# XuyangBai/PointDSC

Hardware: NVIDIA B200
Metric: correspondence-sets/sec (PointDSC.forward, N=1000, B=256) (higher is better)
Workload: dtype fp16 hi/lo split (3 products) with f32 accumulate

## Files before the change

pointdsc_b200/csrc/encoder_tc.cu:

```cuda
#include <cuda_bf16.h>
#include <cuda_fp16.h>
#include <cuda_runtime.h>

#include <cmath>
#include <cstdlib>
#include <cstring>
#include <vector>

#include "common.cuh"
#include "encoder_tc.h"
#include "kernels.h"
#include "tc_attention.cuh"
#include "tc_attention_p.cuh"
#include "tc_chain.cuh"
#include "tc_common.cuh"
#include "tc_ptx.cuh"

namespace pdsc {

template <int FMT>
static void build_image(const float* W, int rows, int K, double scale, uint8_t* dst) {
  const int panels = K / 64;
  const size_t panel_bytes = (size_t)rows * 128;
  uint8_t* hi = dst;
  uint8_t* lo = dst + panels * panel_bytes;
  for (int r = 0; r < rows; ++r)
    for (int k = 0; k < K; ++k) {
      const float x = (float)((double)W[(size_t)r * K + k] * scale);
      const uint16_t h = to_16<FMT>(x);
      const uint16_t l = to_16<FMT>(x - from_16<FMT>(h));
      const size_t off = (size_t)(k / 64) * panel_bytes + sw128_offset((uint32_t)r, (uint32_t)(k % 64));
      std::memcpy(hi + off, &h, 2);
      std::memcpy(lo + off, &l, 2);
    }
}

template <int FMT>
static void build_layer(const TcLayerHost& L, uint8_t* base) {
  build_image<FMT>(L.w1, 128, 128, 1.0, base + kW1);
  build_image<FMT>(L.wq, 128, 128, (double)kQScale, base + kWq);
  build_image<FMT>(L.wk, 128, 128, 1.0, base + kWk);
  build_image<FMT>(L.wv, 128, 128, 1.0, base + kWv);
  build_image<FMT>(L.wm0, 64, 128, 1.0, base + kWm0);
  build_image<FMT>(L.wm1, 64, 64, 1.0, base + kWm1);
  build_image<FMT>(L.wm2, 128, 64, 1.0, base + kWm2);
}

int tc_build_weights(const TcLayerHost* layers, int num_layers, TcWeights* out) {
  tc_free_weights(out);
  const size_t per_fmt = (size_t)num_layers * kLayerBytes;
  std::vector<uint8_t> host(2 * per_fmt, 0);
  for (int fmt = 0; fmt < 2; ++fmt)
    for (int l = 0; l < num_layers; ++l) {
      uint8_t* base = host.data() + fmt * per_fmt + (size_t)l * kLayerBytes;
      const TcLayerHost& L = layers[l];
      if (fmt == kFmtF16) build_layer<kFmtF16>(L, base); else build_layer<kFmtBF16>(L, base);
      float* b = reinterpret_cast<float*>(base + kBias);
      for (int i = 0; i < 128; ++i) {
        b[kB1 + i] = L.b1[i];
        b[kBq + i] = (float)((double)L.bq[i] * (double)kQScale);
        b[kBk + i] = L.bk[i];
        b[kBv + i] = L.bv[i];
        b[kBm2 + i] = L.bm2[i];
      }
      for (int i = 0; i < 64; ++i) {
        b[kBm0 + i] = L.bm0[i];
        b[kBm1 + i] = L.bm1[i];
      }
    }
  cudaError_t err = cudaMalloc(&out->arena, host.size());
  if (err != cudaSuccess) return (int)err;
  err = cudaMemcpy(out->arena, host.data(), host.size(), cudaMemcpyHostToDevice);
  if (err != cudaSuccess) return (int)err;
  out->arena_bytes = host.size();
  out->num_layers = num_layers;
  return 0;
}

void tc_free_weights(TcWeights* w) {
  if (w->arena) cudaFree(w->arena);
  w->arena = nullptr;
  w->arena_bytes = 0;
}

static inline int q_tiles(int N) { return (N + 127) / 128; }
static inline int k_tiles(int N) { return (N + 63) / 64; }

constexpr int kAttnSplitMaxItems = 320;
constexpr size_t kAttnSplitBytes = (size_t)kAttnSplitMaxItems * (65536 + 1024);

size_t tc_scratch_bytes(int B, int N) {
  return ((size_t)B * q_tiles(N) + (size_t)B * k_tiles(N)) * 65536 + 1024 + kAttnSplitBytes;
}

static void attn_split_policy(int B, int N, int num_sms, int* splits, int* TS) {
  const int QT = q_tiles(N), KT = k_tiles(N);
  *splits = 1;
  *TS = KT;
  if (2 * B * QT > num_sms || KT < 4) return;
  const int want = (num_sms + QT - 1) / QT;
  int ts = (KT + want - 1) / want;
  if (ts < 2) ts = 2;
  const int sp = (KT + ts - 1) / ts;
  if (sp < 2 || B * QT * sp > kAttnSplitMaxItems) return;
  *splits = sp;
  *TS = ts;
}

int tc_launches(int num_layers, int B, int N) {
  int splits, ts;
  attn_split_policy(B, N, device_sm_count(), &splits, &ts);
  return 2 + (splits > 1 ? 5 : 4) * num_layers;
}

__global__ void tc_clear_pads_kernel(uint8_t* kvimg, int N, int KT) {
  const int b = blockIdx.x;
  const int first_pad = N & 63;
  if (first_pad == 0) return;
  uint8_t* base = kvimg + ((size_t)b * KT + (KT - 1)) * 65536;
  const int pads = 64 - first_pad;
  for (int t = threadIdx.x; t < pads * 128; t += blockDim.x) {
    const uint32_t n = (uint32_t)(first_pad + t / 128), c = (uint32_t)(t % 128);
    const uint32_t koff = (c >> 6) * 8192u + sw128_offset(n, c & 63u);
    *reinterpret_cast<uint16_t*>(base + koff) = 0;
    *reinterpret_cast<uint16_t*>(base + 16384 + koff) = 0;
    *reinterpret_cast<uint16_t*>(base + 32768 + koff) = 0;
    *reinterpret_cast<uint16_t*>(base + 49152 + koff) = 0;
  }
}

template <int FMT>
__global__ void tc_decode_kernel(const uint8_t* qimg, const uint8_t* kvimg, float* q, float* k, float* v, long long rows,
                                 int N, int QT, int KT, int split) {
  const long long idx = (long long)blockIdx.x * blockDim.x + threadIdx.x;
  const long long row = idx / kC;
  const uint32_t c = (uint32_t)(idx % kC);
  if (row >= rows) return;
  const int b = (int)(row / N), n = (int)(row % N);
  auto rd = [](const uint8_t* p) { return from_16<FMT>(*reinterpret_cast<const uint16_t*>(p)); };
  const uint8_t* qb = qimg + ((size_t)b * QT + (n >> 7)) * 65536;
  const uint32_t qo = (c >> 6) * 16384u + sw128_offset((uint32_t)(n & 127), c & 63u);
  q[idx] = rd(qb + qo) + (split ? rd(qb + 32768 + qo) : 0.f);
  const uint8_t* kb = kvimg + ((size_t)b * KT + (n >> 6)) * 65536;
  const uint32_t ko = (c >> 6) * 8192u + sw128_offset((uint32_t)(n & 63), c & 63u);
  k[idx] = rd(kb + ko) + (split ? rd(kb + 16384 + ko) : 0.f);
  v[idx] = rd(kb + 32768 + ko) + (split ? rd(kb + 49152 + ko) : 0.f);
}

__global__ void tc_unblock_f32_kernel(const float* __restrict__ blocked, float* __restrict__ plain, long long rows) {
  const long long i = (long long)blockIdx.x * blockDim.x + threadIdx.x;
  if (i >= rows * 32) return;
  const long long g = i >> 5;
  const uint32_t piece = (uint32_t)(i & 31);
  reinterpret_cast<float4*>(plain)[i] =
      *reinterpret_cast<const float4*>(reinterpret_cast<const uint8_t*>(blocked) + blocked_f32_offset(g, piece));
}

template <int FMT>
static cudaError_t tc_configure_fmt() {
  cudaError_t e;
  if ((e = ensure_dynamic_smem(reinterpret_cast<const void*>(tc_chain_kernel<kPCQ, FMT>), kChainSmem))) return e;
  if ((e = ensure_dynamic_smem(reinterpret_cast<const void*>(tc_chain_kernel<kKV, FMT>), kChainSmem))) return e;
  if ((e = ensure_dynamic_smem(reinterpret_cast<const void*>(tc_chain_kernel<kMSG, FMT>), kChainSmem))) return e;
  return ensure_dynamic_smem(reinterpret_cast<const void*>(tc_attention_persistent_kernel<FMT>), kAttnPSmem);
}

template <int FMT>
static int tc_encoder_forward_fmt(const TcWeights& w, const TcForwardArgs& a, cudaStream_t st) {
  const long long rows = (long long)a.B * a.N;
  if (rows >= (1LL << 31)) return (int)cudaErrorInvalidValue;
  const int QT = q_tiles(a.N), KT = k_tiles(a.N);
  uint8_t* qimg = static_cast<uint8_t*>(a.scratch);
  qimg = reinterpret_cast<uint8_t*>((reinterpret_cast<uintptr_t>(qimg) + 1023) & ~uintptr_t(1023));
  uint8_t* kvimg = qimg + (size_t)a.B * QT * 65536;
  float* part_o = reinterpret_cast<float*>(kvimg + (size_t)a.B * KT * 65536);
  float* part_ml = part_o + (size_t)kAttnSplitMaxItems * 128 * kC;
  const long long tiles = (rows + 127) / 128;
  const int num_sms = device_sm_count();
  if (num_sms <= 0) return (int)cudaErrorInvalidDevice;
  const int grid = (int)(tiles < num_sms ? tiles : num_sms);
  const uint8_t* arena = static_cast<const uint8_t*>(w.arena) + (size_t)FMT * w.num_layers * kLayerBytes;

  launch_layer0(a.corr_pos, a.l0w, a.l0b, a.feat, rows, a.in_dim, st);
  tc_clear_pads_kernel<<<a.B, 256, 0, st>>>(kvimg, a.N, KT);
  for (int l = 0; l < a.num_layers; ++l) {
    const uint8_t* base = arena + (size_t)l * kLayerBytes;
    ChainArgs c{};
    c.rows = rows; c.N = a.N; c.QT = QT; c.KT = KT; c.split = a.split;
    c.qimg = qimg; c.kvimg = kvimg; c.bias = reinterpret_cast<const float*>(base + kBias);
    c.in = a.feat; c.res = nullptr; c.out_f32 = a.feat1; c.wimg = base + kW1; c.wbytes = 131072;
    c.dbg = (a.timeline && a.debug_layer == l) ? a.timeline : nullptr;
    tc_chain_kernel<kPCQ, FMT><<<grid, kChainThreads, kChainSmem, st>>>(c);
    c.in = a.feat1; c.out_f32 = nullptr; c.wimg = base + kWk; c.wbytes = 131072; c.dbg = nullptr;
    tc_chain_kernel<kKV, FMT><<<grid, kChainThreads, kChainSmem, st>>>(c);
    int splits, ts;
    attn_split_policy(a.B, a.N, num_sms, &splits, &ts);
    AttnArgs at{a.N, a.NS, QT, KT, a.split, qimg, kvimg, a.sc, a.msg,
                (a.timeline && a.debug_layer == l) ? a.timeline + 512 : nullptr, a.B * QT * splits, splits, ts, part_o, part_ml};
    if (a.attn_events) cudaEventRecord(a.attn_events[2 * l], st);
    {
      const int items = at.items;
      tc_attention_persistent_kernel<FMT><<<items < num_sms ? items : num_sms, kAttnThreads, kAttnPSmem, st>>>(at);
      if (splits > 1) tc_attention_merge_kernel<<<a.B * QT * 4, 256, 0, st>>>(part_o, part_ml, a.msg, a.N, QT, splits);
    }
    if (a.attn_events) cudaEventRecord(a.attn_events[2 * l + 1], st);
    if (a.debug_out && a.debug_layer == l) {
      const size_t plane = (size_t)rows * kC;
      tc_unblock_f32_kernel<<<(unsigned)((plane / 4 + 255) / 256), 256, 0, st>>>(a.feat1, a.debug_out, rows);
      tc_decode_kernel<FMT><<<(unsigned)((plane + 255) / 256), 256, 0, st>>>(qimg, kvimg, a.debug_out + plane, a.debug_out + 2 * plane,
                                                                             a.debug_out + 3 * plane, rows, a.N, QT, KT, a.split);
      cudaMemcpyAsync(a.debug_out + 4 * plane, a.msg, plane * sizeof(float), cudaMemcpyDeviceToDevice, st);
    }
    c.in = a.msg; c.res = a.feat1; c.out_f32 = a.feat; c.wimg = base + kWm0; c.wbytes = 81920;
    tc_chain_kernel<kMSG, FMT><<<grid, kChainThreads, kChainSmem, st>>>(c);
    if (a.layer_tap_out && a.layer_tap == l)
      cudaMemcpyAsync(a.layer_tap_out, a.feat, (size_t)rows * kC * sizeof(float), cudaMemcpyDeviceToDevice, st);
  }
  return (int)cudaGetLastError();
}

int tc_encoder_forward(const TcWeights& w, const TcForwardArgs& a, cudaStream_t st) {
  const cudaError_t e = a.fmt == kFmtBF16 ? tc_configure_fmt<kFmtBF16>() : tc_configure_fmt<kFmtF16>();
  if (e != cudaSuccess) return (int)e;
  return a.fmt == kFmtBF16 ? tc_encoder_forward_fmt<kFmtBF16>(w, a, st) : tc_encoder_forward_fmt<kFmtF16>(w, a, st);
}

}
```

pointdsc_b200/csrc/tc_ptx.cuh:

```cuda
#pragma once
#include <cuda_bf16.h>
#include <cuda_fp16.h>
#include <cuda_runtime.h>
#include <stdint.h>

#include <cstdio>

namespace pdsc {
namespace ptx {

__device__ __forceinline__ uint32_t smem_u32(const void* p) { return (uint32_t)__cvta_generic_to_shared(p); }

__device__ __forceinline__ bool elect_one() {
  uint32_t pred = 0, laneid = 0;
  asm volatile(
      "{\n\t.reg .b32 rx;\n\t.reg .pred px;\n\t"
      "elect.sync rx|px, %2;\n\t"
      "@px mov.s32 %1, 1;\n\t"
      "mov.s32 %0, rx;\n\t}"
      : "+r"(laneid), "+r"(pred)
      : "r"(0xFFFFFFFFu));
  return pred != 0;
}

__device__ __forceinline__ void mbar_init(uint32_t bar, uint32_t count) {
  asm volatile("mbarrier.init.shared::cta.b64 [%0], %1;" ::"r"(bar), "r"(count) : "memory");
}
__device__ __forceinline__ void fence_barrier_init() {
  asm volatile("fence.mbarrier_init.release.cluster;" ::: "memory");
}
__device__ __forceinline__ void mbar_arrive(uint32_t bar) {
  asm volatile("mbarrier.arrive.shared::cta.b64 _, [%0];" ::"r"(bar) : "memory");
}
__device__ __forceinline__ void mbar_expect_tx(uint32_t bar, uint32_t bytes) {
  asm volatile("mbarrier.arrive.expect_tx.shared::cta.b64 _, [%0], %1;" ::"r"(bar), "r"(bytes) : "memory");
}
#ifndef PDSC_MBAR_HINT_NS
#define PDSC_MBAR_HINT_NS 1000000u
#endif
constexpr uint32_t kMbarSuspendHintNs = PDSC_MBAR_HINT_NS;
__device__ __forceinline__ bool mbar_try_wait(uint32_t bar, uint32_t parity) {
  uint32_t ok;
  asm volatile(
      "{\n\t.reg .pred p;\n\t"
      "mbarrier.try_wait.parity.shared::cta.b64 p, [%1], %2, %3;\n\t"
      "selp.u32 %0, 1, 0, p;\n\t}"
      : "=r"(ok)
      : "r"(bar), "r"(parity), "r"(kMbarSuspendHintNs)
      : "memory");
  return ok != 0;
}
__device__ __forceinline__ bool mbar_test(uint32_t bar, uint32_t parity) {
  uint32_t ok;
  asm volatile(
      "{\n\t.reg .pred p;\n\t"
      "mbarrier.test_wait.parity.shared::cta.b64 p, [%1], %2;\n\t"
      "selp.u32 %0, 1, 0, p;\n\t}"
      : "=r"(ok)
      : "r"(bar), "r"(parity)
      : "memory");
  return ok != 0;
}
__device__ __forceinline__ void mbar_wait(uint32_t bar, uint32_t parity) {
  if (mbar_try_wait(bar, parity)) return;
  const long long t0 = clock64();
  for (uint32_t tries = 1;; ++tries) {
    if (mbar_try_wait(bar, parity)) return;
    if ((tries & 63u) == 0u && clock64() - t0 > 8000000000LL) {
      printf("pointdsc_b200: mbarrier wait timed out (block %d, thread %d, bar 0x%x, parity %u)\n", blockIdx.x,
             threadIdx.x, bar, parity);
      __trap();
    }
  }
}

__device__ __forceinline__ void bulk_g2s(uint32_t dst_smem, const void* src_gmem, uint32_t bytes, uint32_t bar) {
  asm volatile("cp.async.bulk.shared::cluster.global.mbarrier::complete_tx::bytes [%0], [%1], %2, [%3];" ::"r"(dst_smem),
               "l"(src_gmem), "r"(bytes), "r"(bar)
               : "memory");
}

__device__ __forceinline__ void bulk_s2g(void* dst_gmem, uint32_t src_smem, uint32_t bytes) {
  asm volatile("cp.async.bulk.global.shared::cta.bulk_group [%0], [%1], %2;" ::"l"(__cvta_generic_to_global(dst_gmem)), "r"(src_smem),
               "r"(bytes)
               : "memory");
}
__device__ __forceinline__ void bulk_commit() { asm volatile("cp.async.bulk.commit_group;" ::: "memory"); }
template <int N>
__device__ __forceinline__ void bulk_wait_read() { asm volatile("cp.async.bulk.wait_group.read %0;" ::"n"(N) : "memory"); }
template <int N>
__device__ __forceinline__ void bulk_wait_all() { asm volatile("cp.async.bulk.wait_group %0;" ::"n"(N) : "memory"); }

__device__ __forceinline__ void fence_proxy_async_smem() { asm volatile("fence.proxy.async.shared::cta;" ::: "memory"); }
__device__ __forceinline__ void tc_fence_before() { asm volatile("tcgen05.fence::before_thread_sync;" ::: "memory"); }
__device__ __forceinline__ void tc_fence_after() { asm volatile("tcgen05.fence::after_thread_sync;" ::: "memory"); }

__device__ __forceinline__ void tmem_alloc(uint32_t dst_smem, uint32_t ncols) {
  asm volatile("tcgen05.alloc.cta_group::1.sync.aligned.shared::cta.b32 [%0], %1;" ::"r"(dst_smem), "r"(ncols) : "memory");
  asm volatile("tcgen05.relinquish_alloc_permit.cta_group::1.sync.aligned;" ::: "memory");
}
__device__ __forceinline__ void tmem_dealloc(uint32_t taddr, uint32_t ncols) {
  asm volatile("tcgen05.dealloc.cta_group::1.sync.aligned.b32 %0, %1;" ::"r"(taddr), "r"(ncols) : "memory");
}

__device__ __forceinline__ uint64_t smem_desc_sw128(uint32_t smem_addr) {
  return (uint64_t)((smem_addr >> 4) & 0x3FFFu) | (1ull << 16) | (64ull << 32) | (1ull << 46) | (2ull << 61);
}
__host__ __device__ constexpr uint32_t idesc_f16kind(int M, int N, int fmt) {
  return (1u << 4) | ((uint32_t)fmt << 7) | ((uint32_t)fmt << 10) | ((uint32_t)(N >> 3) << 17) | ((uint32_t)(M >> 4) << 24);
}

__device__ __forceinline__ void mma_bf16(uint32_t d_tmem, uint64_t adesc, uint64_t bdesc, uint32_t idesc, uint32_t accumulate) {
  asm volatile(
      "{\n\t.reg .pred p;\n\t"
      "setp.ne.b32 p, %4, 0;\n\t"
      "tcgen05.mma.cta_group::1.kind::f16 [%0], %1, %2, %3, p;\n\t}"
      ::"r"(d_tmem), "l"(adesc), "l"(bdesc), "r"(idesc), "r"(accumulate)
      : "memory");
}
__device__ __forceinline__ void mma_commit(uint32_t bar) {
  asm volatile("tcgen05.commit.cta_group::1.mbarrier::arrive::one.shared::cluster.b64 [%0];" ::"r"(bar) : "memory");
}

#define PDSC_R32(v)                                                                                               \
  v[0], v[1], v[2], v[3], v[4], v[5], v[6], v[7], v[8], v[9], v[10], v[11], v[12], v[13], v[14], v[15], v[16],  \
      v[17], v[18], v[19], v[20], v[21], v[22], v[23], v[24], v[25], v[26], v[27], v[28], v[29], v[30], v[31]

__device__ __forceinline__ void tmem_ld32(uint32_t taddr, uint32_t (&v)[32]) {
  asm volatile(
      "tcgen05.ld.sync.aligned.32x32b.x32.b32 "
      "{%0, %1, %2, %3, %4, %5, %6, %7, %8, %9, %10, %11, %12, %13, %14, %15, "
      "%16, %17, %18, %19, %20, %21, %22, %23, %24, %25, %26, %27, %28, %29, %30, %31}, [%32];"
      : "=r"(v[0]), "=r"(v[1]), "=r"(v[2]), "=r"(v[3]), "=r"(v[4]), "=r"(v[5]), "=r"(v[6]), "=r"(v[7]), "=r"(v[8]),
        "=r"(v[9]), "=r"(v[10]), "=r"(v[11]), "=r"(v[12]), "=r"(v[13]), "=r"(v[14]), "=r"(v[15]), "=r"(v[16]),
        "=r"(v[17]), "=r"(v[18]), "=r"(v[19]), "=r"(v[20]), "=r"(v[21]), "=r"(v[22]), "=r"(v[23]), "=r"(v[24]),
        "=r"(v[25]), "=r"(v[26]), "=r"(v[27]), "=r"(v[28]), "=r"(v[29]), "=r"(v[30]), "=r"(v[31])
      : "r"(taddr)
      : "memory");
}
__device__ __forceinline__ void tmem_ld_wait() { asm volatile("tcgen05.wait::ld.sync.aligned;" ::: "memory"); }

__device__ __forceinline__ void tmem_st32(uint32_t taddr, const uint32_t (&v)[32]) {
  asm volatile(
      "tcgen05.st.sync.aligned.32x32b.x32.b32 [%0], "
      "{%1, %2, %3, %4, %5, %6, %7, %8, %9, %10, %11, %12, %13, %14, %15, %16, "
      "%17, %18, %19, %20, %21, %22, %23, %24, %25, %26, %27, %28, %29, %30, %31, %32};"
      ::"r"(taddr), "r"(v[0]), "r"(v[1]), "r"(v[2]), "r"(v[3]), "r"(v[4]), "r"(v[5]), "r"(v[6]), "r"(v[7]), "r"(v[8]),
      "r"(v[9]), "r"(v[10]), "r"(v[11]), "r"(v[12]), "r"(v[13]), "r"(v[14]), "r"(v[15]), "r"(v[16]), "r"(v[17]),
      "r"(v[18]), "r"(v[19]), "r"(v[20]), "r"(v[21]), "r"(v[22]), "r"(v[23]), "r"(v[24]), "r"(v[25]), "r"(v[26]),
      "r"(v[27]), "r"(v[28]), "r"(v[29]), "r"(v[30]), "r"(v[31])
      : "memory");
}
__device__ __forceinline__ void tmem_st16(uint32_t taddr, const uint32_t (&v)[16]) {
  asm volatile(
      "tcgen05.st.sync.aligned.32x32b.x16.b32 [%0], "
      "{%1, %2, %3, %4, %5, %6, %7, %8, %9, %10, %11, %12, %13, %14, %15, %16};"
      ::"r"(taddr), "r"(v[0]), "r"(v[1]), "r"(v[2]), "r"(v[3]), "r"(v[4]), "r"(v[5]), "r"(v[6]), "r"(v[7]), "r"(v[8]),
      "r"(v[9]), "r"(v[10]), "r"(v[11]), "r"(v[12]), "r"(v[13]), "r"(v[14]), "r"(v[15])
      : "memory");
}
__device__ __forceinline__ void tmem_st_wait() { asm volatile("tcgen05.wait::st.sync.aligned;" ::: "memory"); }

constexpr int kFmtF16 = 0, kFmtBF16 = 1;

template <int FMT>
__device__ __forceinline__ void split_pair(float a, float b, uint32_t& hi, uint32_t& lo) {
  if (FMT == kFmtBF16) {
    const __nv_bfloat162 h = __floats2bfloat162_rn(a, b);
    const float2 f = __bfloat1622float2(h);
    const __nv_bfloat162 l = __floats2bfloat162_rn(a - f.x, b - f.y);
    hi = *reinterpret_cast<const uint32_t*>(&h);
    lo = *reinterpret_cast<const uint32_t*>(&l);
  } else {
    const __half2 h = __floats2half2_rn(a, b);
    const float2 f = __half22float2(h);
    const __half2 l = __floats2half2_rn(a - f.x, b - f.y);
    hi = *reinterpret_cast<const uint32_t*>(&h);
    lo = *reinterpret_cast<const uint32_t*>(&l);
  }
}
template <int FMT>
__host__ __device__ __forceinline__ uint16_t to_16(float x) {
  if (FMT == kFmtBF16) {
    const __nv_bfloat16 h = __float2bfloat16_rn(x);
    return *reinterpret_cast<const uint16_t*>(&h);
  } else {
    const __half h = __float2half_rn(x);
    return *reinterpret_cast<const uint16_t*>(&h);
  }
}
template <int FMT>
__host__ __device__ __forceinline__ float from_16(uint16_t b) {
  if (FMT == kFmtBF16) {
    return __bfloat162float(*reinterpret_cast<const __nv_bfloat16*>(&b));
  } else {
    return __half2float(*reinterpret_cast<const __half*>(&b));
  }
}

__host__ __device__ __forceinline__ uint32_t sw128_offset(uint32_t row, uint32_t kk) {
  return (row >> 3) * 1024u + (row & 7u) * 128u + ((((kk >> 3) ^ row) & 7u) << 4) + (kk & 7u) * 2u;
}

}
}
```

Baseline: 25580.

## Fuse message MLP with next layer's PCQ projection in 2-CTA cluster kernel

Adds a new cluster-of-two tcgen05 kernel (cta_group::2, M=256) that runs the message MLP chain of layer l together with the next layer's W1 and Wq projections. This replaces separate MSG and PCQ chain launches for every layer except the last, keeping intermediates in TMEM and dropping one launch and one round trip of features per layer. It uses a warp-specialised pipeline with cluster mbarriers, double-buffered TMEM and async bulk stores. The cost is much more complex synchronisation, higher smem use, and a dependence on cluster occupancy.

```diff
diff --git a/pointdsc_b200/csrc/encoder_tc.cu b/pointdsc_b200/csrc/encoder_tc.cu
--- a/pointdsc_b200/csrc/encoder_tc.cu
+++ b/pointdsc_b200/csrc/encoder_tc.cu
@@ -5,6 +5,7 @@
 #include <cmath>
 #include <cstdlib>
 #include <cstring>
+#include <mutex>
 #include <vector>
 
 #include "common.cuh"
@@ -14,6 +15,7 @@
 #include "tc_attention_p.cuh"
 #include "tc_chain.cuh"
 #include "tc_common.cuh"
+#include "tc_pair.cuh"
 #include "tc_ptx.cuh"
 
 namespace pdsc {
@@ -110,7 +112,7 @@
 int tc_launches(int num_layers, int B, int N) {
   int splits, ts;
   attn_split_policy(B, N, device_sm_count(), &splits, &ts);
-  return 2 + (splits > 1 ? 5 : 4) * num_layers;
+  return 3 + (splits > 1 ? 4 : 3) * num_layers;
 }
 
 __global__ void tc_clear_pads_kernel(uint8_t* kvimg, int N, int KT) {
@@ -157,11 +159,31 @@
 }
 
 template <int FMT>
+static int mpq_max_clusters() {
+  static std::mutex mu;
+  static int cached[64] = {};
+  int dev = 0;
+  if (cudaGetDevice(&dev) != cudaSuccess || dev < 0 || dev >= 64) return 0;
+  std::lock_guard<std::mutex> lock(mu);
+  if (cached[dev] == 0) {
+    cudaLaunchConfig_t cfg = {};
+    cfg.gridDim = dim3(2 * device_sm_count(), 1, 1);
+    cfg.blockDim = dim3(kMpqThreads, 1, 1);
+    cfg.dynamicSmemBytes = kMpqSmem;
+    int n = 0;
+    if (cudaOccupancyMaxActiveClusters(&n, tc_mpq_kernel<FMT>, &cfg) != cudaSuccess) return 0;
+    cached[dev] = n;
+  }
+  return cached[dev];
+}
+
+template <int FMT>
 static cudaError_t tc_configure_fmt() {
   cudaError_t e;
   if ((e = ensure_dynamic_smem(reinterpret_cast<const void*>(tc_chain_kernel<kPCQ, FMT>), kChainSmem))) return e;
   if ((e = ensure_dynamic_smem(reinterpret_cast<const void*>(tc_chain_kernel<kKV, FMT>), kChainSmem))) return e;
   if ((e = ensure_dynamic_smem(reinterpret_cast<const void*>(tc_chain_kernel<kMSG, FMT>), kChainSmem))) return e;
+  if ((e = ensure_dynamic_smem(reinterpret_cast<const void*>(tc_mpq_kernel<FMT>), kMpqSmem))) return e;
   return ensure_dynamic_smem(reinterpret_cast<const void*>(tc_attention_persistent_kernel<FMT>), kAttnPSmem);
 }
 
@@ -181,17 +203,26 @@
   const int grid = (int)(tiles < num_sms ? tiles : num_sms);
   const uint8_t* arena = static_cast<const uint8_t*>(w.arena) + (size_t)FMT * w.num_layers * kLayerBytes;
 
+  const long long pair_tiles = (rows + 255) / 256;
+  const int max_clusters = mpq_max_clusters<FMT>();
+  if (max_clusters <= 0) return (int)cudaErrorInvalidConfiguration;
+  const int mpq_grid = 2 * (int)(pair_tiles < max_clusters ? pair_tiles : max_clusters);
+
   launch_layer0(a.corr_pos, a.l0w, a.l0b, a.feat, rows, a.in_dim, st);
   tc_clear_pads_kernel<<<a.B, 256, 0, st>>>(kvimg, a.N, KT);
+  ChainArgs c{};
+  c.rows = rows; c.N = a.N; c.QT = QT; c.KT = KT; c.split = a.split;
+  c.qimg = qimg; c.kvimg = kvimg;
+  {
+    c.bias = reinterpret_cast<const float*>(arena + kBias);
+    c.in = a.feat; c.res = nullptr; c.out_f32 = a.feat1; c.wimg = arena + kW1; c.wbytes = 131072;
+    c.dbg = (a.timeline && a.debug_layer == 0) ? a.timeline : nullptr;
+    tc_chain_kernel<kPCQ, FMT><<<grid, kChainThreads, kChainSmem, st>>>(c);
+  }
   for (int l = 0; l < a.num_layers; ++l) {
     const uint8_t* base = arena + (size_t)l * kLayerBytes;
-    ChainArgs c{};
-    c.rows = rows; c.N = a.N; c.QT = QT; c.KT = KT; c.split = a.split;
-    c.qimg = qimg; c.kvimg = kvimg; c.bias = reinterpret_cast<const float*>(base + kBias);
-    c.in = a.feat; c.res = nullptr; c.out_f32 = a.feat1; c.wimg = base + kW1; c.wbytes = 131072;
-    c.dbg = (a.timeline && a.debug_layer == l) ? a.timeline : nullptr;
-    tc_chain_kernel<kPCQ, FMT><<<grid, kChainThreads, kChainSmem, st>>>(c);
-    c.in = a.feat1; c.out_f32 = nullptr; c.wimg = base + kWk; c.wbytes = 131072; c.dbg = nullptr;
+    c.bias = reinterpret_cast<const float*>(base + kBias);
+    c.in = a.feat1; c.res = nullptr; c.out_f32 = nullptr; c.wimg = base + kWk; c.wbytes = 131072; c.dbg = nullptr;
     tc_chain_kernel<kKV, FMT><<<grid, kChainThreads, kChainSmem, st>>>(c);
     int splits, ts;
     attn_split_policy(a.B, a.N, num_sms, &splits, &ts);
@@ -211,10 +242,16 @@
                                                                              a.debug_out + 3 * plane, rows, a.N, QT, KT, a.split);
       cudaMemcpyAsync(a.debug_out + 4 * plane, a.msg, plane * sizeof(float), cudaMemcpyDeviceToDevice, st);
     }
-    c.in = a.msg; c.res = a.feat1; c.out_f32 = a.feat; c.wimg = base + kWm0; c.wbytes = 81920;
-    tc_chain_kernel<kMSG, FMT><<<grid, kChainThreads, kChainSmem, st>>>(c);
-    if (a.layer_tap_out && a.layer_tap == l)
-      cudaMemcpyAsync(a.layer_tap_out, a.feat, (size_t)rows * kC * sizeof(float), cudaMemcpyDeviceToDevice, st);
+    float* tap = (a.layer_tap_out && a.layer_tap == l) ? a.layer_tap_out : nullptr;
+    if (l + 1 < a.num_layers) {
+      MpqArgs m{rows, a.N, QT, a.split, a.msg, a.feat1, qimg, base, base + kLayerBytes, tap,
+                (a.timeline && a.debug_layer == l + 1) ? a.timeline : nullptr};
+      tc_mpq_kernel<FMT><<<mpq_grid, kMpqThreads, kMpqSmem, st>>>(m);
+    } else {
+      c.in = a.msg; c.res = a.feat1; c.out_f32 = a.feat; c.wimg = base + kWm0; c.wbytes = 81920;
+      tc_chain_kernel<kMSG, FMT><<<grid, kChainThreads, kChainSmem, st>>>(c);
+      if (tap) cudaMemcpyAsync(tap, a.feat, (size_t)rows * kC * sizeof(float), cudaMemcpyDeviceToDevice, st);
+    }
   }
   return (int)cudaGetLastError();
 }
diff --git a/pointdsc_b200/csrc/tc_pair.cuh b/pointdsc_b200/csrc/tc_pair.cuh
--- /dev/null
+++ b/pointdsc_b200/csrc/tc_pair.cuh
@@ -0,0 +1,457 @@
+#pragma once
+#include "tc_chain.cuh"
+
+namespace pdsc {
+
+struct MpqArgs {
+  long long rows;
+  int N, QT, split;
+  const float* msg;
+  float* feat1;
+  uint8_t* qimg;
+  const uint8_t* wl;
+  const uint8_t* wn;
+  float* tap;
+  long long* dbg;
+};
+
+constexpr int kMpqThreads = 512;
+constexpr int kMpqLoaderWarps = 7, kMpqLoaderRows = 19;
+constexpr int kMpA = 0;
+constexpr int kMpWm0 = 65536, kMpWm1 = kMpWm0 + 16384, kMpWm2 = kMpWm1 + 8192, kMpW1 = kMpWm2 + 16384, kMpWq = kMpW1 + 32768;
+constexpr int kMpStage = kMpWq + 32768;
+constexpr int kMpBias = kMpStage + 32768;
+constexpr int kMpBars = kMpBias + 2048;
+constexpr int kMpqSmem = kMpBars + 256;
+static_assert(kMpqSmem <= 232448, "smem map");
+
+template <int KP, int NOUT>
+__device__ __forceinline__ void pair_gemm_ss(uint32_t d_tmem, uint32_t a_hi, uint32_t a_lo, uint32_t a_panel_bytes, uint32_t b_hi,
+                                             uint32_t b_lo, uint32_t b_panel_bytes, int split, int fmt) {
+  const uint32_t idesc = idesc_f16kind(256, NOUT, fmt);
+  constexpr uint32_t kDescHi = 64u | (1u << 14) | (2u << 29);
+  uint32_t acc = 0;
+#pragma unroll
+  for (int t = 0; t < 3; ++t) {
+    if (t > 0 && !split) break;
+    const uint32_t a = (t == 2) ? a_lo : a_hi;
+    const uint32_t b = (t == 1) ? b_lo : b_hi;
+#pragma unroll
+    for (int p = 0; p < KP; ++p) {
+#pragma unroll
+      for (int ks = 0; ks < 4; ++ks) {
+        const uint32_t alo = (((a + p * a_panel_bytes + ks * 32) >> 4) & 0x3FFFu) | (1u << 16);
+        const uint32_t blo = (((b + p * b_panel_bytes + ks * 32) >> 4) & 0x3FFFu) | (1u << 16);
+        asm volatile(
+            "{\n\t.reg .pred p;\n\t.reg .b64 da, db;\n\t"
+            "mov.b64 da, {%1, %5};\n\t"
+            "mov.b64 db, {%2, %5};\n\t"
+            "setp.ne.b32 p, %4, 0;\n\t"
+            "tcgen05.mma.cta_group::2.kind::f16 [%0], da, db, %3, p;\n\t}"
+            ::"r"(d_tmem), "r"(alo), "r"(blo), "r"(idesc), "r"(acc), "r"(kDescHi)
+            : "memory");
+        acc = 1;
+      }
+    }
+  }
+}
+template <int KCH, int NOUT>
+__device__ __forceinline__ void pair_gemm_ts(uint32_t d_tmem, uint32_t a_base, uint32_t b_hi, uint32_t b_lo, uint32_t b_panel_bytes,
+                                             int split, int fmt) {
+  const uint32_t idesc = idesc_f16kind(256, NOUT, fmt);
+  constexpr uint32_t kDescHi = 64u | (1u << 14) | (2u << 29);
+  uint32_t acc = 0;
+#pragma unroll
+  for (int t = 0; t < 3; ++t) {
+    if (t > 0 && !split) break;
+    const uint32_t b = (t == 1) ? b_lo : b_hi;
+#pragma unroll
+    for (int q = 0; q < KCH; ++q) {
+#pragma unroll
+      for (int s = 0; s < 2; ++s) {
+        const int k0 = 32 * q + 16 * s;
+        const uint32_t acol = a_base + 32 * q + (t == 2 ? 16 : 0) + 8 * s;
+        const uint32_t blo = (((b + (k0 >> 6) * b_panel_bytes + ((k0 & 63) >> 4) * 32) >> 4) & 0x3FFFu) | (1u << 16);
+        asm volatile(
+            "{\n\t.reg .pred p;\n\t.reg .b64 db;\n\t"
+            "mov.b64 db, {%2, %5};\n\t"
+            "setp.ne.b32 p, %4, 0;\n\t"
+            "tcgen05.mma.cta_group::2.kind::f16 [%0], [%1], db, %3, p;\n\t}"
+            ::"r"(d_tmem), "r"(acol), "r"(blo), "r"(idesc), "r"(acc), "r"(kDescHi)
+            : "memory");
+        acc = 1;
+      }
+    }
+  }
+}
+
+__device__ __forceinline__ void cp_async_commit() { asm volatile("cp.async.commit_group;" ::: "memory"); }
+template <int N>
+__device__ __forceinline__ void cp_async_wait() { asm volatile("cp.async.wait_group %0;" ::"n"(N) : "memory"); }
+
+template <int FMT>
+__global__ void __cluster_dims__(2, 1, 1) __launch_bounds__(kMpqThreads, 1) tc_mpq_kernel(MpqArgs a) {
+  extern __shared__ __align__(1024) uint8_t smem[];
+  float* bias = reinterpret_cast<float*>(smem + kMpBias);
+  uint64_t* bars = reinterpret_cast<uint64_t*>(smem + kMpBars);
+  uint32_t* tmem_slot = reinterpret_cast<uint32_t*>(bars + 24);
+  const uint32_t s0 = smem_u32(smem);
+  const uint32_t rank = cluster_ctarank();
+  const bool even = rank == 0;
+  const uint32_t bar_w = smem_u32(bars + 0);
+  const uint32_t w_pair = smem_u32(bars + 1);
+  const uint32_t a_ready = smem_u32(bars + 2);
+  const uint32_t a_free = smem_u32(bars + 3);
+  const uint32_t op = smem_u32(bars + 4);
+  const uint32_t d_full = smem_u32(bars + 8);
+  const uint32_t d_free = smem_u32(bars + 18);
+  const int tid = threadIdx.x, warp = tid >> 5, lane = tid & 31;
+  const int N = a.N;
+  const long long rows = a.rows;
+  const int num_pt = (int)((rows + 255) / 256);
+  const int pt0 = (int)(blockIdx.x >> 1), pstride = (int)(gridDim.x >> 1);
+  const bool dbg_cta = a.dbg != nullptr && blockIdx.x == 0;
+
+  if (tid == 0) {
+    if (s0 & 1023u) {
+      printf("pointdsc_b200: dynamic shared memory is not 1024-byte aligned\n");
+      __trap();
+    }
+    mbar_init(bar_w, 1);
+    mbar_init(w_pair, 2);
+    mbar_init(a_ready, 2 * kMpqLoaderWarps * 32);
+    mbar_init(a_free, 1);
+    for (int s = 0; s < 4; ++s) mbar_init(op + 8 * s, 256);
+    for (int i = 0; i < 10; ++i) mbar_init(d_full + 8 * i, 1);
+    mbar_init(d_free, 256); mbar_init(d_free + 8, 256);
+    fence_barrier_init();
+  }
+  if (warp == 15) tmem_alloc2(smem_u32(tmem_slot), 512);
+  {
+    const float* bl = reinterpret_cast<const float*>(a.wl + kBias);
+    const float* bn = reinterpret_cast<const float*>(a.wn + kBias);
+    bias[tid] = tid < 256 ? bl[kBm0 + tid] : bn[kB1 + tid - 256];
+  }
+  tc_fence_before();
+  __syncthreads();
+  cluster_sync();
+  tc_fence_after();
+  const uint32_t tmem = *tmem_slot;
+  if (tid == 0) {
+    mbar_expect_tx(bar_w, 106496u);
+    for (int i = 0; i < 4; ++i) bulk_g2s(s0 + kMpWm0 + 4096 * i, a.wl + kWm0 + 8192 * i + 4096 * rank, 4096, bar_w);
+    for (int i = 0; i < 2; ++i) bulk_g2s(s0 + kMpWm1 + 4096 * i, a.wl + kWm1 + 8192 * i + 4096 * rank, 4096, bar_w);
+    for (int i = 0; i < 2; ++i) bulk_g2s(s0 + kMpWm2 + 8192 * i, a.wl + kWm2 + 16384 * i + 8192 * rank, 8192, bar_w);
+    for (int i = 0; i < 4; ++i) bulk_g2s(s0 + kMpW1 + 8192 * i, a.wn + kW1 + 16384 * i + 8192 * rank, 8192, bar_w);
+    for (int i = 0; i < 4; ++i) bulk_g2s(s0 + kMpWq + 8192 * i, a.wn + kWq + 16384 * i + 8192 * rank, 8192, bar_w);
+  }
+
+  if (warp == 15) {
+    mbar_wait(bar_w, 0);
+    if (elect_one()) mbar_arrive_cluster(w_pair, 0);
+    __syncwarp();
+    if (even) {
+      const bool leader = elect_one();
+      const bool stamp = leader && dbg_cta;
+      mbar_wait_cl(w_pair, 0);
+      const uint32_t w = s0;
+      int it = 0;
+      for (int pt = pt0; pt < num_pt; pt += pstride, ++it) {
+        const int par = it & 1, u = it >> 1;
+        const uint32_t dcol = tmem + (uint32_t)par * 256u;
+        if (stamp) PDSC_STAMP1(a.dbg, it, 0, 0);
+        mbar_wait_cl(a_ready, (uint32_t)(it & 1));
+        if (it >= 2) mbar_wait_cl(d_full + 8 * (2 * 4 + par), (uint32_t)((u - 1) & 1));
+        tc_fence_after();
+        if (stamp) PDSC_STAMP1(a.dbg, it, 0, 1);
+        if (leader) {
+          pair_gemm_ss<2, 64>(dcol, w + kMpA, w + kMpA + 32768, 16384, w + kMpWm0, w + kMpWm0 + 8192, 4096, a.split, FMT);
+          mma_commit2(d_full + 8 * (2 * 0 + par));
+          mma_commit2(a_free);
+        }
+        __syncwarp();
+        mbar_wait_cl(op + 8 * 0, (uint32_t)(it & 1));
+        tc_fence_after();
+        if (leader) {
+          pair_gemm_ts<2, 64>(dcol + 64, dcol, w + kMpWm1, w + kMpWm1 + 4096, 4096, a.split, FMT);
+          mma_commit2(d_full + 8 * (2 * 1 + par));
+        }
+        __syncwarp();
+        mbar_wait_cl(op + 8 * 1, (uint32_t)(it & 1));
+        if (it >= 2) mbar_wait_cl(d_free + 8 * par, (uint32_t)((u - 1) & 1));
+        tc_fence_after();
+        if (leader) {
+          pair_gemm_ts<2, 128>(dcol + 128, dcol + 64, w + kMpWm2, w + kMpWm2 + 8192, 8192, a.split, FMT);
+          mma_commit2(d_full + 8 * (2 * 2 + par));
+        }
+        __syncwarp();
+        if (stamp) PDSC_STAMP1(a.dbg, it, 0, 2);
+      }
+    }
+  } else if (warp >= 8) {
+    const int lw = warp - 8;
+    const bool stamp_ld = dbg_cta && tid == 256;
+    int it = 0;
+    for (int pt = pt0; pt < num_pt; pt += pstride, ++it) {
+      const long long row0 = (long long)(2 * pt + (int)rank) * 128;
+      float4 v[kMpqLoaderRows];
+#pragma unroll
+      for (int i = 0; i < kMpqLoaderRows; ++i) {
+        const int rr = lw + kMpqLoaderWarps * i;
+        const long long grow = row0 + rr;
+        v[i] = (rr < 128 && grow < rows) ? __ldg(reinterpret_cast<const float4*>(a.msg + grow * kC) + lane) : make_float4(0.f, 0.f, 0.f, 0.f);
+      }
+      if (stamp_ld) PDSC_STAMP1(a.dbg, it, 1, 0);
+      if (it > 0) mbar_wait_cl(a_free, (uint32_t)((it - 1) & 1));
+      if (stamp_ld) PDSC_STAMP1(a.dbg, it, 1, 1);
+#pragma unroll
+      for (int i = 0; i < kMpqLoaderRows; ++i) {
+        const int rr = lw + kMpqLoaderWarps * i;
+        if (rr < 128) {
+          uint32_t h0, l0, h1, l1;
+          split_pair<FMT>(v[i].x, v[i].y, h0, l0);
+          split_pair<FMT>(v[i].z, v[i].w, h1, l1);
+          const uint32_t off = (uint32_t)(lane >> 4) * 16384u + sw128_offset((uint32_t)rr, (uint32_t)(lane & 15) * 4u);
+          *reinterpret_cast<uint2*>(smem + kMpA + off) = make_uint2(h0, h1);
+          if (a.split) *reinterpret_cast<uint2*>(smem + kMpA + 32768 + off) = make_uint2(l0, l1);
+        }
+      }
+      fence_proxy_async_smem();
+      mbar_arrive_cluster(a_ready, 0);
+      if (stamp_ld) PDSC_STAMP1(a.dbg, it, 1, 2);
+    }
+  } else if (warp >= 4) {
+    const int q4 = warp & 3;
+    const uint32_t lane_base = ((uint32_t)(q4 * 32)) << 16;
+    const bool stamp = dbg_cta && tid == 128;
+    auto e4 = [&](int itx, int ptx) {
+      const int par = itx & 1, u = itx >> 1;
+      const uint32_t dcol = tmem + lane_base + (uint32_t)par * 256u + 128u;
+      const long long row0 = (long long)(2 * ptx + (int)rank) * 128 + q4 * 32;
+      const int b0 = (int)((unsigned long long)row0 / (unsigned)N);
+      const int n0 = (int)(row0 - (long long)b0 * N);
+      size_t own_off;
+      uint32_t own_x;
+      const bool own_ok = row0 + lane < rows;
+      {
+        int bb, nn;
+        locate_row(b0, n0, lane, N, bb, nn);
+        const uint32_t rit = (uint32_t)(nn & 127);
+        own_off = ((size_t)bb * a.QT + (nn >> 7)) * 65536 + rit * 128u;
+        own_x = rit & 7u;
+      }
+      mbar_wait_cl(d_full + 8 * (2 * 4 + par), (uint32_t)(u & 1));
+      tc_fence_after();
+      if (stamp) PDSC_STAMP1(a.dbg, itx, 3, 2);
+      const float* bvec = bias + 384;
+#pragma unroll 1
+      for (int c = 0; c < 4; ++c) {
+        uint32_t raw[32];
+        tmem_ld32(dcol + 32 * c, raw);
+        tmem_ld_wait();
+        uint32_t hi[16], lo[16];
+#pragma unroll
+        for (int i = 0; i < 32; i += 4) {
+          const float4 bv = *reinterpret_cast<const float4*>(bvec + 32 * c + i);
+          split_pair<FMT>(__uint_as_float(raw[i]) + bv.x, __uint_as_float(raw[i + 1]) + bv.y, hi[i >> 1], lo[i >> 1]);
+          split_pair<FMT>(__uint_as_float(raw[i + 2]) + bv.z, __uint_as_float(raw[i + 3]) + bv.w, hi[(i >> 1) + 1], lo[(i >> 1) + 1]);
+        }
+        if (c == 3) {
+          tc_fence_before();
+          mbar_arrive_cluster(d_free + 8 * par, 0);
+        }
+        const uint32_t poff = (uint32_t)(c >> 1) * 16384u;
+        const uint32_t m = (uint32_t)(c & 1);
+        if (own_ok) {
+          store_image_half(a.qimg + own_off + poff, own_x, m, hi);
+          if (a.split) store_image_half(a.qimg + own_off + poff + 32768u, own_x, m, lo);
+        }
+      }
+      if (stamp) PDSC_STAMP1(a.dbg, itx, 3, 3);
+    };
+    int it = 0;
+    int prev = -1;
+    for (int pt = pt0; pt < num_pt; pt += pstride, ++it) {
+      const int par = it & 1, u = it >> 1;
+      const uint32_t dcol = tmem + lane_base + (uint32_t)par * 256u;
+#pragma unroll 1
+      for (int step = 0; step < 2; ++step) {
+        mbar_wait_cl(d_full + 8 * (2 * step + par), (uint32_t)(u & 1));
+        tc_fence_after();
+        if (stamp) PDSC_STAMP1(a.dbg, it, 3, step);
+        const uint32_t dstep = step == 0 ? 0u : 64u;
+        const float* bvec = bias + (step == 0 ? 0 : 64);
+#pragma unroll 1
+        for (int c0 = 0; c0 < 64; c0 += 32) {
+          uint32_t raw[32];
+          tmem_ld32(dcol + dstep + c0, raw);
+          tmem_ld_wait();
+          uint32_t hi[16], lo[16];
+#pragma unroll
+          for (int i = 0; i < 32; i += 4) {
+            const float4 bv = *reinterpret_cast<const float4*>(bvec + c0 + i);
+            split_pair<FMT>(fmaxf(__uint_as_float(raw[i]) + bv.x, 0.f), fmaxf(__uint_as_float(raw[i + 1]) + bv.y, 0.f), hi[i >> 1], lo[i >> 1]);
+            split_pair<FMT>(fmaxf(__uint_as_float(raw[i + 2]) + bv.z, 0.f), fmaxf(__uint_as_float(raw[i + 3]) + bv.w, 0.f), hi[(i >> 1) + 1],
+                            lo[(i >> 1) + 1]);
+          }
+          tmem_st16(dcol + dstep + c0, hi);
+          if (a.split) tmem_st16(dcol + dstep + c0 + 16, lo);
+        }
+        tmem_st_wait();
+        tc_fence_before();
+        mbar_arrive_cluster(op + 8 * step, 0);
+      }
+      if (prev >= 0) e4(it - 1, prev);
+      prev = pt;
+    }
+    if (prev >= 0) e4(it - 1, prev);
+  } else {
+    const int q4 = warp & 3;
+    const uint32_t lane_base = ((uint32_t)(q4 * 32)) << 16;
+    uint8_t* stage = smem + kMpStage + warp * 8192;
+    const uint32_t stage_row = smem_u32(stage) + (uint32_t)lane * 128u;
+    const bool stamp = dbg_cta && tid == 0;
+    const bool issuer = even && warp == 0;
+    const uint32_t dcol0 = tmem;
+    bool w_seen = false;
+    auto issue_back = [&](uint32_t bar, int itx, uint32_t dc, int step) {
+      if (!w_seen) {
+        mbar_wait_cl(w_pair, 0);
+        w_seen = true;
+      }
+      mbar_wait_cl(bar, (uint32_t)(itx & 1));
+      tc_fence_after();
+      if (elect_one()) {
+        if (step == 3) pair_gemm_ts<4, 128>(dc, dc + 128, s0 + kMpW1, s0 + kMpW1 + 16384, 8192, a.split, FMT);
+        else pair_gemm_ts<4, 128>(dc + 128, dc, s0 + kMpWq, s0 + kMpWq + 16384, 8192, a.split, FMT);
+        mma_commit2(d_full + 8 * (2 * step + (itx & 1)));
+      }
+      __syncwarp();
+    };
+    auto prefetch_res = [&](int ptx) {
+      const long long tx = 2 * (long long)ptx + (int)rank;
+      if (ptx < num_pt && tx * 128 + q4 * 32 + lane < rows) {
+        const uint8_t* r = reinterpret_cast<const uint8_t*>(a.feat1) + (size_t)tx * 65536 + (size_t)(q4 * 32 + lane) * 128;
+#pragma unroll
+        for (int c = 0; c < 4; ++c) asm volatile("prefetch.global.L2 [%0];" ::"l"(__cvta_generic_to_global(r + (size_t)c * 16384)));
+      }
+    };
+    prefetch_res(pt0);
+    int it = 0;
+    for (int pt = pt0; pt < num_pt; pt += pstride, ++it) {
+      const int par = it & 1, u = it >> 1;
+      const uint32_t dcol = tmem + lane_base + (uint32_t)par * 256u;
+      prefetch_res(pt + pstride);
+      const long long tile = 2 * pt + (int)rank;
+      const long long row0 = tile * 128 + q4 * 32;
+      const long long g = row0 + lane;
+      const bool own_ok = g < rows;
+      const uint8_t* res_row = reinterpret_cast<const uint8_t*>(a.feat1) + (size_t)tile * 65536 + (size_t)(q4 * 32 + lane) * 128;
+      auto fetch_res = [&](int c) {
+#pragma unroll
+        for (int q = 0; q < 8; ++q)
+          cp_async16(stage_row + (uint32_t)(c & 1) * 4096u + (uint32_t)q * 16u,
+                     own_ok ? (const void*)(res_row + (size_t)c * 16384 + q * 16) : (const void*)a.feat1, own_ok ? 16u : 0u);
+        cp_async_commit();
+      };
+      if (lane == 0) bulk_wait_read<0>();
+      __syncwarp();
+      fetch_res(0);
+      fetch_res(1);
+      mbar_wait_cl(d_full + 8 * (2 * 2 + par), (uint32_t)(u & 1));
+      tc_fence_after();
+      if (stamp) PDSC_STAMP1(a.dbg, it, 2, 0);
+#pragma unroll 1
+      for (int c = 0; c < 4; ++c) {
+        if (c < 3) cp_async_wait<1>(); else cp_async_wait<0>();
+        float res[32];
+#pragma unroll
+        for (int q = 0; q < 8; ++q) {
+          const float4 r4 = *reinterpret_cast<const float4*>(stage + (c & 1) * 4096 + lane * 128 + ((q ^ (lane & 7)) << 4));
+          res[4 * q] = r4.x; res[4 * q + 1] = r4.y; res[4 * q + 2] = r4.z; res[4 * q + 3] = r4.w;
+        }
+        if (c + 2 < 4) fetch_res(c + 2);
+        uint32_t raw[32];
+        tmem_ld32(dcol + 128 + 32 * c, raw);
+        tmem_ld_wait();
+#pragma unroll
+        for (int i = 0; i < 32; ++i) res[i] += __uint_as_float(raw[i]) + bias[128 + 32 * c + i];
+        if (a.tap && own_ok) {
+          float* tp = a.tap + g * kC + 32 * c;
+#pragma unroll
+          for (int k = 0; k < 4; ++k)
+            st_global_v8(tp + 8 * k, __float_as_uint(res[8 * k]), __float_as_uint(res[8 * k + 1]), __float_as_uint(res[8 * k + 2]),
+                         __float_as_uint(res[8 * k + 3]), __float_as_uint(res[8 * k + 4]), __float_as_uint(res[8 * k + 5]),
+                         __float_as_uint(res[8 * k + 6]), __float_as_uint(res[8 * k + 7]));
+        }
+        uint32_t hi[16], lo[16];
+#pragma unroll
+        for (int i = 0; i < 16; ++i) split_pair<FMT>(res[2 * i], res[2 * i + 1], hi[i], lo[i]);
+        tmem_st16(dcol + 128 + 32 * c, hi);
+        if (a.split) tmem_st16(dcol + 128 + 32 * c + 16, lo);
+      }
+      tmem_st_wait();
+      tc_fence_before();
+      mbar_arrive_cluster(op + 8 * 2, 0);
+      if (stamp) PDSC_STAMP1(a.dbg, it, 2, 1);
+      if (issuer) issue_back(op + 8 * 2, it, dcol0 + (uint32_t)par * 256u, 3);
+      mbar_wait_cl(d_full + 8 * (2 * 3 + par), (uint32_t)(u & 1));
+      tc_fence_after();
+      if (stamp) PDSC_STAMP1(a.dbg, it, 2, 2);
+#pragma unroll 1
+      for (int cc = 0; cc < 4; ++cc) {
+        const int c0 = 32 * cc;
+        uint32_t raw[32];
+        tmem_ld32(dcol + c0, raw);
+        tmem_ld_wait();
+        uint32_t xb[32];
+#pragma unroll
+        for (int i = 0; i < 32; i += 4) {
+          const float4 bv = *reinterpret_cast<const float4*>(bias + 256 + c0 + i);
+          xb[i] = __float_as_uint(fmaxf(__uint_as_float(raw[i]) + bv.x, 0.f));
+          xb[i + 1] = __float_as_uint(fmaxf(__uint_as_float(raw[i + 1]) + bv.y, 0.f));
+          xb[i + 2] = __float_as_uint(fmaxf(__uint_as_float(raw[i + 2]) + bv.z, 0.f));
+          xb[i + 3] = __float_as_uint(fmaxf(__uint_as_float(raw[i + 3]) + bv.w, 0.f));
+        }
+        {
+          uint32_t hi[16], lo[16];
+#pragma unroll
+          for (int i = 0; i < 16; ++i) split_pair<FMT>(__uint_as_float(xb[2 * i]), __uint_as_float(xb[2 * i + 1]), hi[i], lo[i]);
+          tmem_st16(dcol + c0, hi);
+          if (a.split) tmem_st16(dcol + c0 + 16, lo);
+        }
+        if (cc == 3) {
+          tmem_st_wait();
+          tc_fence_before();
+          mbar_arrive_cluster(op + 8 * 3, 0);
+          if (stamp) PDSC_STAMP1(a.dbg, it, 2, 3);
+        }
+        {
+          uint8_t* buf = stage + (cc & 1) * 4096;
+          if (lane == 0) bulk_wait_read<1>();
+          __syncwarp();
+#pragma unroll
+          for (int q = 0; q < 8; ++q)
+            *reinterpret_cast<uint4*>(buf + lane * 128 + ((q ^ (lane & 7)) << 4)) = make_uint4(xb[4 * q], xb[4 * q + 1], xb[4 * q + 2], xb[4 * q + 3]);
+          fence_proxy_async_smem();
+          __syncwarp();
+          const long long valid = rows - row0;
+          if (lane == 0 && valid > 0) {
+            bulk_s2g(reinterpret_cast<uint8_t*>(a.feat1) + (size_t)tile * 65536 + (size_t)cc * 16384 + (size_t)q4 * 4096, smem_u32(buf),
+                     (uint32_t)(valid < 32 ? valid : 32) * 128u);
+            bulk_commit();
+          }
+        }
+      }
+      if (issuer) issue_back(op + 8 * 3, it, dcol0 + (uint32_t)par * 256u, 4);
+      if (stamp) PDSC_STAMP1(a.dbg, it, 2, 4);
+    }
+    if (lane == 0) bulk_wait_all<0>();
+  }
+  tc_fence_before();
+  __syncthreads();
+  cluster_sync();
+  if (warp == 15) tmem_dealloc2(tmem, 512);
+}
+
+}
diff --git a/pointdsc_b200/csrc/tc_ptx.cuh b/pointdsc_b200/csrc/tc_ptx.cuh
--- a/pointdsc_b200/csrc/tc_ptx.cuh
+++ b/pointdsc_b200/csrc/tc_ptx.cuh
@@ -101,6 +101,57 @@
 }
 __device__ __forceinline__ void tmem_dealloc(uint32_t taddr, uint32_t ncols) {
   asm volatile("tcgen05.dealloc.cta_group::1.sync.aligned.b32 %0, %1;" ::"r"(taddr), "r"(ncols) : "memory");
+}
+
+__device__ __forceinline__ uint32_t cluster_ctarank() {
+  uint32_t r;
+  asm volatile("mov.u32 %0, %%cluster_ctarank;" : "=r"(r));
+  return r;
+}
+__device__ __forceinline__ void cluster_sync() {
+  asm volatile("barrier.cluster.arrive.release.aligned;\n\tbarrier.cluster.wait.acquire.aligned;" ::: "memory");
+}
+__device__ __forceinline__ void tmem_alloc2(uint32_t dst_smem, uint32_t ncols) {
+  asm volatile("tcgen05.alloc.cta_group::2.sync.aligned.shared::cta.b32 [%0], %1;" ::"r"(dst_smem), "r"(ncols) : "memory");
+  asm volatile("tcgen05.relinquish_alloc_permit.cta_group::2.sync.aligned;" ::: "memory");
+}
+__device__ __forceinline__ void tmem_dealloc2(uint32_t taddr, uint32_t ncols) {
+  asm volatile("tcgen05.dealloc.cta_group::2.sync.aligned.b32 %0, %1;" ::"r"(taddr), "r"(ncols) : "memory");
+}
+__device__ __forceinline__ void mbar_arrive_cluster(uint32_t bar, uint32_t rank) {
+  asm volatile(
+      "{\n\t.reg .b32 ra;\n\t"
+      "mapa.shared::cluster.u32 ra, %0, %1;\n\t"
+      "mbarrier.arrive.release.cluster.shared::cluster.b64 _, [ra];\n\t}" ::"r"(bar), "r"(rank)
+      : "memory");
+}
+__device__ __forceinline__ bool mbar_try_wait_cl(uint32_t bar, uint32_t parity) {
+  uint32_t ok;
+  asm volatile(
+      "{\n\t.reg .pred p;\n\t"
+      "mbarrier.try_wait.parity.acquire.cluster.shared::cta.b64 p, [%1], %2, %3;\n\t"
+      "selp.u32 %0, 1, 0, p;\n\t}"
+      : "=r"(ok)
+      : "r"(bar), "r"(parity), "r"(kMbarSuspendHintNs)
+      : "memory");
+  return ok != 0;
+}
+__device__ __forceinline__ void mbar_wait_cl(uint32_t bar, uint32_t parity) {
+  if (mbar_try_wait_cl(bar, parity)) return;
+  const long long t0 = clock64();
+  for (uint32_t tries = 1;; ++tries) {
+    if (mbar_try_wait_cl(bar, parity)) return;
+    if ((tries & 63u) == 0u && clock64() - t0 > 8000000000LL) {
+      printf("pointdsc_b200: cluster mbarrier wait timed out (block %d, thread %d, bar 0x%x, parity %u)\n", blockIdx.x,
+             threadIdx.x, bar, parity);
+      __trap();
+    }
+  }
+}
+__device__ __forceinline__ void mma_commit2(uint32_t bar) {
+  asm volatile("tcgen05.commit.cta_group::2.mbarrier::arrive::one.shared::cluster.multicast::cluster.b64 [%0], %1;" ::"r"(bar),
+               "h"((uint16_t)3)
+               : "memory");
 }
 
 __device__ __forceinline__ uint64_t smem_desc_sw128(uint32_t smem_addr) {
```

New measurement: 25980 (median of 6 runs). 1.02x the previous value.
